# rsokolovskii/fl_scaling_sc_ldpc

Measured on AMD Instinct MI355X. Metric: MC codeword trials/sec, (4,8) SC-LDPC L=50 N=1000 eps=0.48 full BP, higher is better.
Workload: dtype u32

## Files before the change

fl_scaling_sc_ldpc_amd/csrc/philox.h:

```cpp
#pragma once
#include <cstdint>

namespace scldpc_dev {

__device__ __forceinline__ void philox4x32_10(uint32_t c0, uint32_t c1, uint32_t c2, uint32_t c3,
                                              uint32_t k0, uint32_t k1, uint32_t (&out)[4])
{
#pragma unroll
    for (int r = 0; r < 10; r++) {
        const uint64_t p0 = (uint64_t)0xD2511F53u * c0, p1 = (uint64_t)0xCD9E8D57u * c2;
        c0 = __builtin_amdgcn_bitop3_b32((uint32_t)(p1 >> 32), c1, k0, 0x96); c1 = (uint32_t)p1;
        c2 = __builtin_amdgcn_bitop3_b32((uint32_t)(p0 >> 32), c3, k1, 0x96); c3 = (uint32_t)p0;
        k0 += 0x9E3779B9u; k1 += 0xBB67AE85u;
    }
    out[0] = c0; out[1] = c1; out[2] = c2; out[3] = c3;
}

}
```

fl_scaling_sc_ldpc_amd/csrc/sampler_v2.hip:

```cpp
#include "common.h"
#include "kernel_util.h"
#include "philox.h"
#include <algorithm>
#include <cstdlib>

namespace {

using scldpc_dev::philox4x32_10;
using scldpc_dev::wave_inclusive_scan;

constexpr int kThreads = 1024;
constexpr int kWaves = kThreads / 64;
constexpr int kMaxDoped = 32;
constexpr int kWorkCap = 1024;

struct S2Args {
    int L, cns_pos, vns_pos, n, S, D, nb, nw;
    int ntrials;
    int force_exact;
    int ndoped;
    int doped[kMaxDoped];
    uint32_t seed_lo, seed_hi;
    unsigned long long trial0;
    uint32_t thresh;
    int off_gpk, off_fix, off_stage, off_wsum;
    uint16_t *vn_adj16;
    uint16_t *cn_adj16;
    uint32_t *chan;
};

template <int KMAX, int ROWS, int CNMODE, bool PERSIST = false>
__global__ __launch_bounds__(kThreads, KMAX == 1 ? 8 : 4) __attribute__((amdgpu_num_sgpr(72))) void sample_philox_v2_kernel(const S2Args a)
{
    constexpr int DV = 4, DC_SHIFT = 3, E = 4 * KMAX;
    constexpr int LG = ROWS == 1 ? 10 : ROWS == 2 ? 11 : ROWS == 4 ? 12 : 13;
    constexpr int KSHIFT = 32 - LG - 2;
    constexpr bool INCL = KMAX == 1;
    static_assert(ROWS * kThreads == (1 << LG) && (INCL ? ROWS <= 4 : ROWS == 8), "ROWS is 1, 2, 4 (KMAX 1) or 8 (KMAX 2)");
    extern __shared__ uint32_t lds[];
    uint32_t *hist = lds;
    uint32_t *gpk = lds + a.off_gpk;
    uint16_t *fix = reinterpret_cast<uint16_t *>(lds + a.off_fix);
    uint16_t *stage = reinterpret_cast<uint16_t *>(lds + a.off_stage);
    uint32_t *wsum = lds + a.off_wsum;
    uint32_t *wl = wsum + 32;

    const int tid = threadIdx.x, lane = tid & 63, wave = tid >> 6;
    const int S = a.S, nb = a.nb;
    const int ncalls = S >> 2;
    bool own[KMAX];
#pragma unroll
    for (int k = 0; k < KMAX; k++) own[k] = tid + k * kThreads < ncalls;
    auto sock = [&](int e) { return (uint32_t)((tid + (e >> 2) * kThreads) * 4 + (e & 3)); };
    auto stage_entry = [&](int p, uint32_t sck) -> uint16_t {
        const int u = (int)(sck & 3u), t = (int)(sck >> 2);
        if ((unsigned)(p - u) >= (unsigned)a.L) return (uint16_t)0xFFFFu;
        return CNMODE == 1 ? (uint16_t)((p - u) * a.vns_pos + t) : (uint16_t)sck;
    };

    auto nib_sum = [](uint32_t x) {
        const uint32_t v = (x & 0x0F0Fu) + ((x >> 4) & 0x0F0Fu);
        return (v + (v >> 8)) & 0xFFu;
    };
    auto load_words = [&](uint32_t (&x)[ROWS]) {
        if constexpr (ROWS % 4 == 0) {
#pragma unroll
            for (int r = 0; r < ROWS / 4; r++) {
                const uint4 q = reinterpret_cast<const uint4 *>(hist)[tid * (ROWS / 4) + r];
                x[4 * r] = q.x; x[4 * r + 1] = q.y; x[4 * r + 2] = q.z; x[4 * r + 3] = q.w;
            }
        } else if constexpr (ROWS == 2) { const uint2 q = reinterpret_cast<const uint2 *>(hist)[tid]; x[0] = q.x; x[1] = q.y; }
        else x[0] = hist[tid];
    };
    auto store_words = [&](const uint32_t (&x)[ROWS]) {
        if constexpr (ROWS % 4 == 0) {
#pragma unroll
            for (int r = 0; r < ROWS / 4; r++)
                reinterpret_cast<uint4 *>(hist)[tid * (ROWS / 4) + r] = make_uint4(x[4 * r], x[4 * r + 1], x[4 * r + 2], x[4 * r + 3]);
        } else if constexpr (ROWS == 2) reinterpret_cast<uint2 *>(hist)[tid] = make_uint2(x[0], x[1]);
        else hist[tid] = x[0];
    };
    STAMP_DECL
    for (int b = tid; b < nb; b += kThreads) hist[b] = 0;
    if (tid == 0) { wsum[kWaves] = 0; wsum[kWaves + 1] = 0; }
    __syncthreads();
    auto sample_trial = [&](const int tr) {
    const unsigned long long trial = a.trial0 + (unsigned long long)tr;
    const uint32_t t_lo = (uint32_t)trial, t_hi = (uint32_t)(trial >> 32);
    uint32_t rowP[KMAX], rowQ[KMAX], rowR[KMAX];
#pragma unroll
    for (int k = 0; k < KMAX; k++) rowP[k] = rowQ[k] = rowR[k] = 0;
    uint32_t nxt[E];
#pragma unroll
    for (int k = 0; k < KMAX; k++) {
        uint32_t r[4] = {0, 0, 0, 0};
        if (own[k]) philox4x32_10((uint32_t)(tid + k * kThreads), 0u, t_lo, t_hi, a.seed_lo, a.seed_hi, r);
#pragma unroll
        for (int u = 0; u < 4; u++) nxt[4 * k + u] = r[u];
    }
    for (int p = 0; p < a.D; p++) {
        STAMP(0);
        uint32_t key[E], slot[E], crowded = 0;
        auto word_of = [](uint32_t k) { return (k >> KSHIFT) & ~3u; };
        auto nib_of = [](uint32_t k) { return (k >> (KSHIFT - 2)) & 12u; };
#pragma unroll
        for (int e = 0; e < E; e++) {
            key[e] = nxt[e];
            const uint32_t sh = nib_of(key[e]);
            uint32_t *w = reinterpret_cast<uint32_t *>(reinterpret_cast<char *>(hist) + word_of(key[e]));
            slot[e] = (atomicAdd(w, (own[e >> 2] ? 1u : 0u) << sh) >> sh) & 0xFu;
            if constexpr (!INCL) crowded = max(crowded, slot[e]);
        }
        if (!INCL && crowded >= 15u) wsum[kWaves + 1] = 1u;
        __syncthreads();
        STAMP(1);

        bool ranked;
        if constexpr (INCL) {
            uint32_t x[ROWS], t20[ROWS], tot20 = 0;
            load_words(x);
#pragma unroll
            for (int r = 0; r < ROWS; r++) {
                x[r] *= 0x111110u;
                t20[r] = x[r] & 0xF00000u;
                tot20 += t20[r];
            }
            const uint32_t tot = tot20 >> 20, inc = wave_inclusive_scan(tot);
            if (lane == 63) wsum[wave] = inc;
            __syncthreads();
            uint32_t winc = lane < kWaves ? wsum[lane] : 0u;
            const uint32_t wt = winc;
            winc += (uint32_t)__builtin_amdgcn_update_dpp(0, (int)winc, 0x111, 0xF, 0xF, false);
            winc += (uint32_t)__builtin_amdgcn_update_dpp(0, (int)winc, 0x112, 0xF, 0xF, false);
            winc += (uint32_t)__builtin_amdgcn_update_dpp(0, (int)winc, 0x114, 0xF, 0xF, false);
            winc += (uint32_t)__builtin_amdgcn_update_dpp(0, (int)winc, 0x118, 0xF, 0xF, false);
            ranked = __builtin_amdgcn_readlane((int)winc, kWaves - 1) == S;
            uint32_t pre20 = (inc - tot + (uint32_t)__builtin_amdgcn_readlane((int)(winc - wt), wave)) << 20;
#pragma unroll
            for (int r = 0; r < ROWS; r++) {
                x[r] = (x[r] & 0xFFFF0u) | pre20;
                pre20 += t20[r];
            }
            store_words(x);
        } else {
            uint32_t x[ROWS], v[ROWS], tot = 0;
            load_words(x);
#pragma unroll
            for (int r = 0; r < ROWS; r++) v[r] = 0;
            if constexpr (ROWS % 2 == 0) {
#pragma unroll
                for (int r = 0; r < ROWS; r += 2) {
                    const uint32_t y = x[r] | (x[r + 1] << 16);
                    const uint32_t sb = (y & 0x0F0F0F0Fu) + ((y >> 4) & 0x0F0F0F0Fu);
                    v[r] = (sb & 0xFFu) + ((sb >> 8) & 0xFFu);
                    v[r + 1] = ((sb >> 16) & 0xFFu) + (sb >> 24);
                    tot += v[r] + v[r + 1];
                }
            } else {
                static_assert(ROWS == 1 || ROWS % 2 == 0, "ROWS is 1, 2, 4 or 8");
                v[0] = nib_sum(x[0]);
                tot = v[0];
            }
            const uint32_t inc = wave_inclusive_scan(tot);
            if (lane == 63) wsum[wave] = inc;
            __syncthreads();
            const uint32_t wt = lane < kWaves ? wsum[lane] : 0u;
            const uint32_t winc = wave_inclusive_scan(wt);
            uint32_t pre = inc - tot + (uint32_t)__builtin_amdgcn_readlane((int)(winc - wt), wave);
#pragma unroll
            for (int r = 0; r < ROWS; r++) { x[r] |= pre << 16; pre += v[r]; }
            store_words(x);
        }
        __syncthreads();
        if constexpr (!INCL) ranked = wsum[kWaves + 1] == 0u;
        STAMP(2);

        if (ranked) {
            uint32_t rk[E], g0a[E], g1a[E];
            bool st[E];
            if constexpr (INCL) {
                uint32_t h[E];
#pragma unroll
                for (int e = 0; e < E; e++) h[e] = *reinterpret_cast<const uint32_t *>(reinterpret_cast<const char *>(hist) + word_of(key[e]));
#pragma unroll
                for (int e = 0; e < E; e++) {
                    const uint32_t t = h[e] >> nib_of(key[e]), pre = h[e] >> 20;
                    g0a[e] = pre + (t & 0xFu);
                    g1a[e] = pre + ((t >> 4) & 0xFu);
                    rk[e] = g0a[e] + slot[e];
                    st[e] = own[e >> 2] && ((g0a[e] ^ (g1a[e] - 1u)) >> DC_SHIFT) != 0u;
                }
            } else {
                uint32_t h[E];
#pragma unroll
                for (int e = 0; e < E; e++) h[e] = hist[own[e >> 2] ? (key[e] >> KSHIFT) >> 2 : 0u];
#pragma unroll
                for (int e = 0; e < E; e++) {
                    const uint32_t k4 = ((key[e] >> KSHIFT) & 3u) * 4u, x = h[e];
                    const uint32_t below = x & ((1u << k4) - 1u);
                    g0a[e] = (x >> 16) + (below & 0xFu) + ((below >> 4) & 0xFu) + ((below >> 8) & 0xFu);
                    g1a[e] = g0a[e] + ((x >> k4) & 0xFu);
                    rk[e] = g0a[e] + slot[e];
                    st[e] = own[e >> 2] && ((g1a[e] - 1u) >> DC_SHIFT) != (g0a[e] >> DC_SHIFT);
                }
            }
            if constexpr (INCL) {
                unsigned long long vote[E], anyv = 0;
                int total = 0;
#pragma unroll
                for (int e = 0; e < E; e++) { vote[e] = __builtin_amdgcn_ballot_w64(st[e]); anyv |= vote[e]; total += __builtin_popcountll(vote[e]); }
                if (anyv) {
                    int base = 0;
                    if (lane == 0) base = atomicAdd(reinterpret_cast<int *>(&wsum[kWaves]), total);
                    base = __builtin_amdgcn_readfirstlane(base);
                    const bool fits = base + total <= kWorkCap;
#pragma unroll
                    for (int e = 0; e < E; e++) {
                        if (st[e]) {
                            const uint32_t w = __builtin_amdgcn_mbcnt_hi((uint32_t)(vote[e] >> 32),
                                                                         __builtin_amdgcn_mbcnt_lo((uint32_t)vote[e], (uint32_t)base));
                            const uint32_t pk = (key[e] << LG) | sock(e);
                            gpk[rk[e]] = pk;
                            if (fits) { wl[2 * w] = g0a[e] | (g1a[e] << 16); wl[2 * w + 1] = pk; }
                        }
                        base += __builtin_popcountll(vote[e]);
                    }
                }
            } else {
                uint32_t smask = 0;
#pragma unroll
                for (int e = 0; e < E; e++) smask |= (st[e] ? 1u : 0u) << e;
                while (smask) {
                    const uint32_t e = (uint32_t)__ffs((int)smask) - 1u;
                    smask &= smask - 1u;
                    uint32_t ky = key[0], r0 = rk[0], g0 = g0a[0], g1 = g1a[0];
#pragma unroll
                    for (int f = 1; f < E; f++)
                        if (e == (uint32_t)f) { ky = key[f]; r0 = rk[f]; g0 = g0a[f]; g1 = g1a[f]; }
                    const uint32_t pk = (ky << LG) | (uint32_t)((tid + (int)(e >> 2) * kThreads) * 4 + (int)(e & 3u));
                    gpk[r0] = pk;
                    const int w = atomicAdd(reinterpret_cast<int *>(&wsum[kWaves]), 1);
                    if (w < kWorkCap) { wl[2 * w] = g0 | (g1 << 16); wl[2 * w + 1] = pk; }
                }
            }
#pragma unroll
            for (int k = 0; k < KMAX; k++) {
                if (!own[k]) continue;
                uint2 v;
                v.x = (rk[4 * k] >> DC_SHIFT) | ((rk[4 * k + 1] >> DC_SHIFT) << 16);
                v.y = (rk[4 * k + 2] >> DC_SHIFT) | ((rk[4 * k + 3] >> DC_SHIFT) << 16);
                reinterpret_cast<uint2 *>(fix)[tid + k * kThreads] = v;
            }
            if constexpr (CNMODE != 0) {
#pragma unroll
                for (int k = 0; k < KMAX; k++) {
                    if (!own[k]) continue;
#pragma unroll
                    for (int u = 0; u < 4; u++) stage[rk[4 * k + u]] = stage_entry(p, sock(4 * k + u));
                }
            }
        }
        __syncthreads();
        STAMP(3);

        {
            uint32_t z[ROWS];
#pragma unroll
            for (int r = 0; r < ROWS; r++) z[r] = 0;
            store_words(z);
            int nwork = (int)wsum[kWaves];
            const bool exact = !ranked || nwork > kWorkCap || a.force_exact == p || a.force_exact == -2;
            if (exact) {
                asm volatile("; ledger: cold");
                nwork = 0;
#pragma unroll
                for (int e = 0; e < E; e++) if (own[e >> 2]) gpk[sock(e)] = key[e];
                __syncthreads();
                uint32_t xr[E];
#pragma unroll
                for (int e = 0; e < E; e++) xr[e] = 0;
                for (int s2 = 0; s2 < S; s2++) {
                    const uint32_t k2 = gpk[s2];
#pragma unroll
                    for (int e = 0; e < E; e++) xr[e] += (k2 < key[e]) || (k2 == key[e] && (uint32_t)s2 < sock(e));
                }
#pragma unroll
                for (int k = 0; k < KMAX; k++) {
                    if (!own[k]) continue;
                    uint2 v;
                    v.x = (xr[4 * k] >> DC_SHIFT) | ((xr[4 * k + 1] >> DC_SHIFT) << 16);
                    v.y = (xr[4 * k + 2] >> DC_SHIFT) | ((xr[4 * k + 3] >> DC_SHIFT) << 16);
                    reinterpret_cast<uint2 *>(fix)[tid + k * kThreads] = v;
                    if constexpr (CNMODE != 0) {
#pragma unroll
                        for (int u = 0; u < 4; u++) stage[xr[4 * k + u]] = stage_entry(p, sock(4 * k + u));
                    }
                }
            }
            for (int w = tid; w < nwork; w += kThreads) {
                const uint32_t ea = wl[2 * w], pk = wl[2 * w + 1];
                uint32_t r = ea & 0xFFFFu;
#pragma unroll 1
                for (uint32_t m = ea & 0xFFFFu; m < (ea >> 16); m++) r += gpk[m] < pk;
                const uint32_t sck = pk & ((1u << LG) - 1u);
                if constexpr (CNMODE != 0) stage[r] = stage_entry(p, sck);
                fix[sck] = (uint16_t)(r >> DC_SHIFT);
            }
        }
        if (p + 1 < a.D) {
            uint32_t k_lo = a.seed_lo, k_hi = a.seed_hi;
            asm volatile("" : "+s"(k_lo), "+s"(k_hi));
#pragma unroll
            for (int k = 0; k < KMAX; k++) {
                uint32_t r[4] = {0, 0, 0, 0};
                if (own[k]) philox4x32_10((uint32_t)(tid + k * kThreads), (uint32_t)(p + 1), t_lo, t_hi, k_lo, k_hi, r);
#pragma unroll
                for (int u = 0; u < 4; u++) nxt[4 * k + u] = r[u];
            }
        }
        __syncthreads();
        if (tid == 0) { wsum[kWaves] = 0; wsum[kWaves + 1] = 0; }
        STAMP(4);

        const int qpos = p - (DV - 1);
#pragma unroll
        for (int k = 0; k < KMAX; k++) {
            uint2 c = make_uint2(0u, 0u);
            if (own[k]) c = reinterpret_cast<const uint2 *>(fix)[tid + k * kThreads];
            if (qpos >= 0 && own[k]) {
                const size_t j = (size_t)tr * a.n + (size_t)qpos * a.vns_pos + (size_t)(tid + k * kThreads);
                uint2 v;
                v.x = rowP[k];
                v.y = (rowR[k] >> 16) | (c.y & 0xFFFF0000u);
                reinterpret_cast<uint2 *>(a.vn_adj16)[j] = v;
            }
            rowP[k] = rowQ[k];
            rowQ[k] = (rowR[k] & 0xFFFFu) | (c.x & 0xFFFF0000u);
            rowR[k] = (c.x & 0xFFFFu) | (c.y << 16);
        }
        if constexpr (CNMODE != 0) {
            uint2 *dst = reinterpret_cast<uint2 *>(a.cn_adj16) + ((size_t)tr * a.D + p) * (size_t)(S >> 2);
            const uint2 *src = reinterpret_cast<const uint2 *>(stage);
            for (int w = tid; w < (S >> 2); w += kThreads) dst[w] = src[w];
        }
        STAMP(5);
    }

    uint32_t *chan = a.chan + (size_t)tr * a.nw;
    for (int w = tid; w < a.nw; w += kThreads) {
        uint32_t word = 0;
#pragma unroll
        for (int c = 0; c < 8; c++) {
            uint32_t r[4];
            philox4x32_10((uint32_t)(w * 8 + c), 0x80000000u, t_lo, t_hi, a.seed_lo, a.seed_hi, r);
#pragma unroll
            for (int u = 0; u < 4; u++) word |= (uint32_t)((r[u] >> 1) < a.thresh) << (c * 4 + u);
        }
        const int j0 = w * 32;
        if (j0 + 32 > a.n) word &= (1u << (a.n - j0)) - 1u;
        for (int d = 0; d < a.ndoped; d++) {
            const int lo = max(a.doped[d] * a.vns_pos, j0) - j0, hi = min((a.doped[d] + 1) * a.vns_pos, j0 + 32) - j0;
            if (lo < hi) word &= ~(((hi - lo) == 32 ? 0xFFFFFFFFu : ((1u << (hi - lo)) - 1u)) << lo);
        }
        chan[w] = word;
    }
    STAMP(6);
    };
    if constexpr (PERSIST) {
        for (int tr = blockIdx.x; tr < a.ntrials; tr += gridDim.x) {
            sample_trial(tr);
            __syncthreads();
        }
    } else {
        sample_trial((int)blockIdx.x);
    }
    STAMP_FLUSH();
}


__device__ __forceinline__ uint32_t wl_entry_vn(const S2Args &a, int p, uint32_t sck)
{
    return (uint32_t)((p - (int)(sck & 3u)) * a.vns_pos + (int)(sck >> 2));
}

template <int LG, int CNMODE>
__global__ __launch_bounds__(kThreads, 8) __attribute__((amdgpu_num_sgpr(72))) void sample_philox_v3_kernel(const S2Args a)
{
    constexpr int DV = 4, DC_SHIFT = 3, E = 4;
    constexpr int NB = 1 << LG, ROWS = NB / kThreads;
    constexpr int KSHIFT = 32 - LG - 2;
    constexpr uint32_t LOWMASK = (1u << KSHIFT) - 1u;
    constexpr int SBITS = LG;
    static_assert(ROWS == 1 || ROWS == 2 || ROWS == 4, "one Philox call per thread: at most 4096 sockets per position");
    extern __shared__ uint32_t lds[];
    uint32_t *hist0 = lds;
    uint32_t *gpk = lds + a.off_gpk;
    uint16_t *fix = reinterpret_cast<uint16_t *>(lds + a.off_fix);
    uint16_t *stage = reinterpret_cast<uint16_t *>(lds + a.off_stage);
    uint32_t *wsum = lds + a.off_wsum;
    uint32_t *wl = wsum + 32;

    const int tid = threadIdx.x, lane = tid & 63, wave = tid >> 6;
    const int S = a.S;
    const bool own = tid < (S >> 2);
    const unsigned long long trial = a.trial0 + blockIdx.x;
    const uint32_t t_lo = (uint32_t)trial, t_hi = (uint32_t)(trial >> 32);
    const int tr = blockIdx.x;

    STAMP_DECL
    for (int b = tid; b < 2 * NB; b += kThreads) hist0[b] = 0;
    if (tid < 32) wsum[tid] = 0;
    __syncthreads();

    uint32_t rowP = 0, rowQ = 0, rowR = 0;
    uint32_t key[E] = {0, 0, 0, 0}, slot[E] = {0, 0, 0, 0};
    uint32_t ent0 = CNMODE == 1 ? (uint32_t)tid : (uint32_t)(4 * tid);
    uint32_t vV = (uint32_t)a.vns_pos;
    asm volatile("" : "+v"(vV));

    for (int p = 0; p <= a.D; p++) {
        uint32_t *hc = hist0 + (p & 1) * NB, *hp = hist0 + ((p & 1) ^ 1) * NB;
        const bool live = p < a.D;
        STAMP(0);
        if (p > 0) {
            int nwork = (int)wsum[16];
            const bool exact = wsum[18 + ((p - 1) & 1)] != 0u || nwork > kWorkCap || a.force_exact == p - 1 || a.force_exact == -2;
            if (exact) {
                uint32_t k2[4] = {0, 0, 0, 0};
                uint32_t f_lo = a.seed_lo, f_hi = a.seed_hi;
                asm volatile("" : "+s"(f_lo), "+s"(f_hi));
                if (own) philox4x32_10((uint32_t)tid, (uint32_t)(p - 1), t_lo, t_hi, f_lo, f_hi, k2);
                if (own) { gpk[4 * tid] = k2[0]; gpk[4 * tid + 1] = k2[1]; gpk[4 * tid + 2] = k2[2]; gpk[4 * tid + 3] = k2[3]; }
                __syncthreads();
                uint32_t xr[4] = {0, 0, 0, 0};
                for (int s2 = 0; s2 < S; s2++) {
                    const uint32_t kk = gpk[s2];
#pragma unroll
                    for (int u = 0; u < 4; u++) xr[u] += (kk < k2[u]) || (kk == k2[u] && s2 < 4 * tid + u);
                }
                if (own) {
                    uint2 v;
                    v.x = (xr[0] >> DC_SHIFT) | ((xr[1] >> DC_SHIFT) << 16);
                    v.y = (xr[2] >> DC_SHIFT) | ((xr[3] >> DC_SHIFT) << 16);
                    reinterpret_cast<uint2 *>(fix)[tid] = v;
                    if constexpr (CNMODE != 0) {
#pragma unroll
                        for (int u = 0; u < 4; u++) {
                            const int pu = p - 1 - u;
                            stage[xr[u]] = (unsigned)pu < (unsigned)a.L ? (uint16_t)(CNMODE == 1 ? pu * a.vns_pos + tid : 4 * tid + u) : (uint16_t)0xFFFFu;
                        }
                    }
                }
                nwork = 0;
            }
            for (int w = tid; w < nwork; w += kThreads) {
                const uint32_t ea = wl[2 * w], pk = wl[2 * w + 1];
                const uint32_t g0 = ea & 0xFFFFu, cnt = (ea >> 16) & 0xFu, sl = (ea >> 20) & 0xFu;
                uint32_t r = g0;
                for (uint32_t m = 0; m < cnt; m++)
                    if (m != sl) r += gpk[g0 + m] < pk;
                const uint32_t sck = pk & ((1u << SBITS) - 1u);
                if constexpr (CNMODE != 0) stage[r] = (uint16_t)(ea >> 24 ? 0xFFFFu : (CNMODE == 1 ? wl_entry_vn(a, p - 1, sck) : sck));
                fix[sck] = (uint16_t)(r >> DC_SHIFT);
            }
            {
                if constexpr (ROWS == 4) reinterpret_cast<uint4 *>(hp)[tid] = make_uint4(0u, 0u, 0u, 0u);
                else if constexpr (ROWS == 2) reinterpret_cast<uint2 *>(hp)[tid] = make_uint2(0u, 0u);
                else hp[tid] = 0u;
            }
        }
        STAMP(1);
        if (live) {
            {
                uint32_t k_lo = a.seed_lo, k_hi = a.seed_hi;
                asm volatile("" : "+s"(k_lo), "+s"(k_hi));
                uint32_t r[4] = {0, 0, 0, 0};
                if (own) philox4x32_10((uint32_t)tid, (uint32_t)p, t_lo, t_hi, k_lo, k_hi, r);
#pragma unroll
                for (int u = 0; u < 4; u++) key[u] = r[u];
            }
            uint32_t crowded = 0;
#pragma unroll
            for (int e = 0; e < E; e++) {
                const uint32_t boff = (key[e] >> KSHIFT) & ~3u, sh = (key[e] >> (KSHIFT - 2)) & 12u;
                const uint32_t old = atomicAdd(reinterpret_cast<uint32_t *>(reinterpret_cast<char *>(hc) + boff), (own ? 16u : 0u) << sh);
                slot[e] = (old >> (sh + 4u)) & 0xFu;
                crowded |= slot[e] + 1u;
            }
            if (crowded & 16u) wsum[18 + (p & 1)] = 1u;
        }
        STAMP(2);
        __syncthreads();
        STAMP(3);
        if (tid == 0) { wsum[16] = 0; wsum[18 + ((p & 1) ^ 1)] = 0; }
        if (live) {
            uint32_t x[ROWS], tot = 0, over = 0;
            if constexpr (ROWS == 4) { const uint4 q = reinterpret_cast<const uint4 *>(hc)[tid]; x[0] = q.x; x[1] = q.y; x[2] = q.z; x[3] = q.w; }
            else if constexpr (ROWS == 2) { const uint2 q = reinterpret_cast<const uint2 *>(hc)[tid]; x[0] = q.x; x[1] = q.y; }
            else x[0] = hc[tid];
            uint32_t v[ROWS];
#pragma unroll
            for (int r = 0; r < ROWS; r++) {
                const uint32_t y = x[r] * 0x1111u;
                const uint32_t sb = (x[r] & 0x0F0F0u) + ((x[r] >> 4) & 0x0F0F0u);
                v[r] = ((sb + (sb >> 8)) >> 4) & 0xFFu;
                over |= v[r];
                x[r] = y & 0xFFFF0u;
                tot += v[r];
            }
            if (over & ~15u) wsum[18 + (p & 1)] = 1u;
            const uint32_t inc = wave_inclusive_scan(tot);
            uint32_t pre = inc - tot;
#pragma unroll
            for (int r = 0; r < ROWS; r++) { x[r] |= pre << 20; pre += v[r]; }
            if constexpr (ROWS == 4) reinterpret_cast<uint4 *>(hc)[tid] = make_uint4(x[0], x[1], x[2], x[3]);
            else if constexpr (ROWS == 2) reinterpret_cast<uint2 *>(hc)[tid] = make_uint2(x[0], x[1]);
            else hc[tid] = x[0];
            if (lane == 63) wsum[wave] = inc;
        }
        if (p > 0) {
            const int pp = p - 1, qpos = pp - (DV - 1);
            uint2 c = make_uint2(0u, 0u);
            if (own) c = reinterpret_cast<const uint2 *>(fix)[tid];
            if (qpos >= 0 && own) {
                const size_t j = (size_t)tr * a.n + (size_t)qpos * a.vns_pos + (size_t)tid;
                uint2 vv;
                vv.x = rowP;
                vv.y = (rowR >> 16) | (c.y & 0xFFFF0000u);
                reinterpret_cast<uint2 *>(a.vn_adj16)[j] = vv;
            }
            rowP = rowQ;
            rowQ = (rowR & 0xFFFFu) | (c.x & 0xFFFF0000u);
            rowR = (c.x & 0xFFFFu) | (c.y << 16);
            if constexpr (CNMODE != 0) {
                uint2 *dst = reinterpret_cast<uint2 *>(a.cn_adj16) + ((size_t)tr * a.D + pp) * (size_t)(S >> 2);
                const uint2 *src = reinterpret_cast<const uint2 *>(stage);
                if (own) dst[tid] = src[tid];
            }
        }
        STAMP(4);
        __syncthreads();
        STAMP(5);
        if (live && wsum[18 + (p & 1)] == 0u) {
            const uint32_t wt = lane < kWaves ? wsum[lane] : 0u;
            uint32_t wi = wt;
            wi += (uint32_t)__builtin_amdgcn_update_dpp(0, (int)wi, 0x111, 0xF, 0xF, false);
            wi += (uint32_t)__builtin_amdgcn_update_dpp(0, (int)wi, 0x112, 0xF, 0xF, false);
            wi += (uint32_t)__builtin_amdgcn_update_dpp(0, (int)wi, 0x114, 0xF, 0xF, false);
            wi += (uint32_t)__builtin_amdgcn_update_dpp(0, (int)wi, 0x118, 0xF, 0xF, false);
            const uint32_t wex = wi - wt;
            uint32_t h[E], wb[E], rk[E], g0a[E], cnta[E];
#pragma unroll
            for (int e = 0; e < E; e++) h[e] = *reinterpret_cast<const uint32_t *>(reinterpret_cast<const char *>(hc) + ((key[e] >> KSHIFT) & ~3u));
#pragma unroll
            for (int e = 0; e < E; e++) wb[e] = (uint32_t)__builtin_amdgcn_ds_bpermute((int)((key[e] >> 26) & 0x3Cu), (int)wex);
            bool st[E];
            bool anyst = false;
#pragma unroll
            for (int e = 0; e < E; e++) {
                const uint32_t t1 = h[e] >> ((key[e] >> (KSHIFT - 2)) & 12u);
                const uint32_t excl = t1 & 15u, incl = (t1 >> 4) & 15u;
                g0a[e] = (h[e] >> 20) + wb[e] + excl;
                cnta[e] = incl - excl;
                rk[e] = g0a[e] + slot[e];
                st[e] = own && ((g0a[e] ^ (g0a[e] + cnta[e] - 1u)) >> DC_SHIFT) != 0u;
                anyst = anyst || st[e];
            }
            if (own) {
                uint2 vv;
                vv.x = (rk[0] >> DC_SHIFT) | ((rk[1] >> DC_SHIFT) << 16);
                vv.y = (rk[2] >> DC_SHIFT) | ((rk[3] >> DC_SHIFT) << 16);
                reinterpret_cast<uint2 *>(fix)[tid] = vv;
            }
            const bool edge = p < DV - 1 || p >= a.L;
            if constexpr (CNMODE != 0) {
                if (own) {
                    uint32_t ent[E];
                    ent[0] = ent0;
#pragma unroll
                    for (int u = 1; u < 4; u++) ent[u] = CNMODE == 1 ? ent[u - 1] - vV : ent[u - 1] + 1u;
                    if (!edge) {
#pragma unroll
                        for (int u = 0; u < 4; u++) stage[rk[u]] = (uint16_t)ent[u];
                    } else {
#pragma unroll
                        for (int u = 0; u < 4; u++) stage[rk[u]] = (unsigned)(p - u) < (unsigned)a.L ? (uint16_t)ent[u] : (uint16_t)0xFFFFu;
                    }
                }
            }
            if (__builtin_amdgcn_ballot_w64(anyst)) {
                unsigned long long vote[E];
                int total = 0;
#pragma unroll
                for (int e = 0; e < E; e++) { vote[e] = __builtin_amdgcn_ballot_w64(st[e]); total += __builtin_popcountll(vote[e]); }
                int base = 0;
                if (lane == 0) base = atomicAdd(reinterpret_cast<int *>(&wsum[16]), total);
                base = __builtin_amdgcn_readfirstlane(base);
#pragma unroll
                for (int e = 0; e < E; e++) {
                    if (st[e]) {
                        const int w = base + (int)__builtin_amdgcn_mbcnt_hi((uint32_t)(vote[e] >> 32), __builtin_amdgcn_mbcnt_lo((uint32_t)vote[e], 0u));
                        const uint32_t pk = ((key[e] & LOWMASK) << SBITS) | (uint32_t)(4 * tid + e);
                        gpk[g0a[e] + slot[e]] = pk;
                        const uint32_t none = CNMODE != 0 && edge && !((unsigned)(p - e) < (unsigned)a.L) ? 1u : 0u;
                        if (w < kWorkCap) { wl[2 * w] = g0a[e] | (cnta[e] << 16) | (slot[e] << 20) | (none << 24); wl[2 * w + 1] = pk; }
                    }
                    base += __builtin_popcountll(vote[e]);
                }
            }
        }
        if constexpr (CNMODE == 1) ent0 += vV;
        STAMP(6);
        __syncthreads();
        STAMP(7);
    }

    uint32_t *chan = a.chan + (size_t)tr * a.nw;
    for (int w = tid; w < a.nw; w += kThreads) {
        uint32_t word = 0;
        uint32_t c_lo = a.seed_lo, c_hi = a.seed_hi;
        asm volatile("" : "+s"(c_lo), "+s"(c_hi));
#pragma unroll
        for (int c = 0; c < 8; c++) {
            uint32_t r[4];
            philox4x32_10((uint32_t)(w * 8 + c), 0x80000000u, t_lo, t_hi, c_lo, c_hi, r);
#pragma unroll
            for (int u = 0; u < 4; u++) word |= (uint32_t)((r[u] >> 1) < a.thresh) << (c * 4 + u);
        }
        const int j0 = w * 32;
        if (j0 + 32 > a.n) word &= (1u << (a.n - j0)) - 1u;
        for (int d = 0; d < a.ndoped; d++) {
            const int lo = max(a.doped[d] * a.vns_pos, j0) - j0, hi = min((a.doped[d] + 1) * a.vns_pos, j0 + 32) - j0;
            if (lo < hi) word &= ~(((hi - lo) == 32 ? 0xFFFFFFFFu : ((1u << (hi - lo)) - 1u)) << lo);
        }
        chan[w] = word;
    }
    STAMP(8);
    STAMP_FLUSH();
}

int launch_v2(const char *who, int cnmode, const scldpc_code_params *p, uint64_t seed, uint64_t trial0, int32_t ntrials,
              double eps, int32_t ndoped, const int32_t *doped_positions, uint16_t *d_vn_adj16, uint16_t *d_table,
              uint32_t *d_chan_bits, void *stream)
{
    if (ntrials < 0 || (ntrials > 0 && (!d_vn_adj16 || !d_chan_bits)))
        return scldpc::set_error(SCLDPC_ERR_BAD_ARG, "%s: null buffer or negative ntrials", who);
    if (ndoped < 0 || ndoped > kMaxDoped || (ndoped > 0 && !doped_positions))
        return scldpc::set_error(SCLDPC_ERR_BAD_ARG, "%s: 0 <= ndoped <= %d", who, kMaxDoped);
    if (!(eps >= 0.0 && eps <= 1.0))
        return scldpc::set_error(SCLDPC_ERR_BAD_ARG, "%s: eps=%g outside [0,1]", who, eps);
    if (ntrials == 0) return SCLDPC_OK;
    if (!d_table) cnmode = 0;

    S2Args a{};
    a.L = p->L; a.cns_pos = p->cns_pos; a.vns_pos = p->vns_pos;
    a.n = scldpc::n_of(p); a.S = p->cns_pos * p->dc; a.D = p->L + p->dv - 1; a.nw = scldpc::nw_of(p);
    int lg = 10;
    while ((1 << lg) < a.S) lg++;
    a.nb = 1 << lg;
    a.ndoped = ndoped;
    for (int d = 0; d < ndoped; d++) {
        if (doped_positions[d] < 0 || doped_positions[d] >= p->L)
            return scldpc::set_error(SCLDPC_ERR_BAD_ARG, "doped position %d outside [0,%d)", doped_positions[d], p->L);
        a.doped[d] = doped_positions[d];
    }
    a.seed_lo = (uint32_t)seed; a.seed_hi = (uint32_t)(seed >> 32);
    a.trial0 = trial0;
    {
        const double x = eps * 2147483647.0;
        double c = (double)(uint64_t)x;
        if (c < x) c += 1.0;
        a.thresh = (uint32_t)c;
    }
    const char *gen_env = getenv("SCLDPC_SAMPLER_GEN");
    const bool v3 = a.nb <= 4 * kThreads && gen_env && atoi(gen_env) == 3;
    int off = ((v3 ? 2 : 1) * a.nb + 3) & ~3;
    a.off_gpk = off;   off += (a.S + 3) & ~3;
    a.off_fix = off;   off += (a.S / 2 + 3) & ~3;
    a.off_stage = off; off += cnmode ? (a.S / 2 + 3) & ~3 : 0;
    a.off_wsum = off;  off += 32 + 2 * kWorkCap;
    size_t lds_bytes = 4u * (size_t)off;
    lds_bytes = std::min(lds_bytes + scldpc::debug_lds_pad("SAMPLER"), std::max(lds_bytes, (size_t)scldpc::kMaxLdsBytes));
    if (lds_bytes > (size_t)scldpc::kMaxLdsBytes)
        return scldpc::set_error(SCLDPC_ERR_TOO_LARGE, "%s: %zu bytes of LDS per trial", who, lds_bytes);
    a.vn_adj16 = d_vn_adj16; a.cn_adj16 = d_table; a.chan = d_chan_bits;
    a.ntrials = ntrials;
    a.force_exact = -1;
    if (const char *v = getenv("SCLDPC_DEBUG_SAMPLER_EXACT_POS")) a.force_exact = atoi(v);

    using Kern = void (*)(const S2Args);
    static const Kern table[4][3] = {
        {sample_philox_v2_kernel<1, 1, 0>, sample_philox_v2_kernel<1, 1, 1>, sample_philox_v2_kernel<1, 1, 2>},
        {sample_philox_v2_kernel<1, 2, 0>, sample_philox_v2_kernel<1, 2, 1>, sample_philox_v2_kernel<1, 2, 2>},
        {sample_philox_v2_kernel<1, 4, 0>, sample_philox_v2_kernel<1, 4, 1>, sample_philox_v2_kernel<1, 4, 2>},
        {sample_philox_v2_kernel<2, 8, 0>, sample_philox_v2_kernel<2, 8, 1>, sample_philox_v2_kernel<2, 8, 2>},
    };
    const int rows = a.nb / kThreads;
    static const Kern table3[3][3] = {
        {sample_philox_v3_kernel<10, 0>, sample_philox_v3_kernel<10, 1>, sample_philox_v3_kernel<10, 2>},
        {sample_philox_v3_kernel<11, 0>, sample_philox_v3_kernel<11, 1>, sample_philox_v3_kernel<11, 2>},
        {sample_philox_v3_kernel<12, 0>, sample_philox_v3_kernel<12, 1>, sample_philox_v3_kernel<12, 2>},
    };
    const int grid = v3 ? ntrials : scldpc::debug_grid("SAMPLER", ntrials);
    Kern kern = v3 ? table3[lg - 10][cnmode] : table[rows == 1 ? 0 : rows == 2 ? 1 : rows == 4 ? 2 : 3][cnmode];
    if (grid < ntrials && rows == 4 && cnmode == 1) kern = sample_philox_v2_kernel<1, 4, 1, true>;
    else if (grid < ntrials) return scldpc::set_error(SCLDPC_ERR_BAD_ARG, "SCLDPC_DEBUG_GRID_SAMPLER: only the <1,4,1> kernel has a persistent form");
    if (int rc_ = scldpc::allow_max_lds(reinterpret_cast<const void *>(kern))) return rc_;
    hipLaunchKernelGGL(kern, dim3(grid), dim3(kThreads), lds_bytes, static_cast<hipStream_t>(stream), a);
    SCLDPC_HIP_CHECK(hipGetLastError());
    return SCLDPC_OK;
}

bool v2_shape(const scldpc_code_params *p)
{
    if (scldpc::check_params(p)) return false;
    const int S = p->cns_pos * p->dc;
    return p->dv == 4 && p->dc == 8 && (S & 3) == 0 && S <= 8192 && p->vns_pos * p->dv == S;
}

}

extern "C" int scldpc_sample_philox_cn16_supported(const scldpc_code_params *p)
{
    return v2_shape(p) && scldpc::n_of(p) < 65535;
}

extern "C" int scldpc_sample_philox_sock16_supported(const scldpc_code_params *p)
{
    return v2_shape(p);
}

extern "C" int scldpc_sample_philox_device_cn16(const scldpc_code_params *p, uint64_t seed, uint64_t trial0,
                                                int32_t ntrials, double eps, int32_t ndoped,
                                                const int32_t *doped_positions, uint16_t *d_vn_adj16,
                                                uint16_t *d_cn_adj16, uint32_t *d_chan_bits, void *stream)
{
    const char *who = "scldpc_sample_philox_device_cn16";
    if (int rc = scldpc::check_params(p)) return rc;
    if (!scldpc_sample_philox_cn16_supported(p))
        return scldpc::set_error(SCLDPC_ERR_TOO_LARGE, "%s: takes dv = 4, dc = 8, at most 8192 sockets per position and "
                                 "fewer than 65535 VNs (got dv=%d dc=%d cns_pos=%d n=%d)", who, p->dv, p->dc, p->cns_pos,
                                 scldpc::n_of(p));
    return launch_v2(who, 1, p, seed, trial0, ntrials, eps, ndoped, doped_positions, d_vn_adj16, d_cn_adj16, d_chan_bits,
                     stream);
}

extern "C" int scldpc_sample_philox_device_sock16(const scldpc_code_params *p, uint64_t seed, uint64_t trial0,
                                                  int32_t ntrials, double eps, int32_t ndoped,
                                                  const int32_t *doped_positions, uint16_t *d_vn_adj16,
                                                  uint16_t *d_cn_sock16, uint32_t *d_chan_bits, void *stream)
{
    const char *who = "scldpc_sample_philox_device_sock16";
    if (int rc = scldpc::check_params(p)) return rc;
    if (!scldpc_sample_philox_sock16_supported(p))
        return scldpc::set_error(SCLDPC_ERR_TOO_LARGE, "%s: takes dv = 4, dc = 8 and at most 8192 sockets per position "
                                 "(got dv=%d dc=%d cns_pos=%d)", who, p->dv, p->dc, p->cns_pos);
    return launch_v2(who, 2, p, seed, trial0, ntrials, eps, ndoped, doped_positions, d_vn_adj16, d_cn_sock16, d_chan_bits,
                     stream);
}
```

Baseline: 1.214 million.

## Hoist per-thread Philox prefix rounds and share trial-uniform rounds across positions

Splits Philox4x32-10 into a per-thread prefix (depends only on thread counter, trial and key), a wave-uniform part that depends on the position counter, and a tail for rounds 3-9. The prefix is computed once per trial and reused across all D positions, so each position pays for fewer per-thread rounds while producing the same random stream. It also makes the LDS layout offsets compile-time for the inclusive path, and uses a hand-written ds_add_rtn with a ballot-masked worklist append. It adds a raw asm LDS atomic with an explicit waitcnt and changes the host layout sizing, which must stay consistent with the constexpr offsets.

```diff
diff --git a/fl_scaling_sc_ldpc_amd/csrc/philox.h b/fl_scaling_sc_ldpc_amd/csrc/philox.h
--- a/fl_scaling_sc_ldpc_amd/csrc/philox.h
+++ b/fl_scaling_sc_ldpc_amd/csrc/philox.h
@@ -1,17 +1,86 @@
 #pragma once
 #include <cstdint>
 
+#if defined(__HIPCC__) || defined(__CUDACC__)
+#define SCLDPC_PHILOX_HD __host__ __device__ __forceinline__
+#else
+#define SCLDPC_PHILOX_HD inline
+#endif
+
 namespace scldpc_dev {
 
-__device__ __forceinline__ void philox4x32_10(uint32_t c0, uint32_t c1, uint32_t c2, uint32_t c3,
-                                              uint32_t k0, uint32_t k1, uint32_t (&out)[4])
+constexpr uint32_t kPhiloxM0 = 0xD2511F53u, kPhiloxM1 = 0xCD9E8D57u;
+constexpr uint32_t kPhiloxW0 = 0x9E3779B9u, kPhiloxW1 = 0xBB67AE85u;
+
+SCLDPC_PHILOX_HD uint32_t philox_xor3(uint32_t a, uint32_t b, uint32_t c)
+{
+#if defined(__HIP_DEVICE_COMPILE__)
+    return __builtin_amdgcn_bitop3_b32(a, b, c, 0x96);
+#else
+    return a ^ b ^ c;
+#endif
+}
+
+SCLDPC_PHILOX_HD void philox4x32_10(uint32_t c0, uint32_t c1, uint32_t c2, uint32_t c3,
+                                    uint32_t k0, uint32_t k1, uint32_t (&out)[4])
 {
 #pragma unroll
     for (int r = 0; r < 10; r++) {
-        const uint64_t p0 = (uint64_t)0xD2511F53u * c0, p1 = (uint64_t)0xCD9E8D57u * c2;
-        c0 = __builtin_amdgcn_bitop3_b32((uint32_t)(p1 >> 32), c1, k0, 0x96); c1 = (uint32_t)p1;
-        c2 = __builtin_amdgcn_bitop3_b32((uint32_t)(p0 >> 32), c3, k1, 0x96); c3 = (uint32_t)p0;
-        k0 += 0x9E3779B9u; k1 += 0xBB67AE85u;
+        const uint64_t p0 = (uint64_t)kPhiloxM0 * c0, p1 = (uint64_t)kPhiloxM1 * c2;
+        c0 = philox_xor3((uint32_t)(p1 >> 32), c1, k0); c1 = (uint32_t)p1;
+        c2 = philox_xor3((uint32_t)(p0 >> 32), c3, k1); c3 = (uint32_t)p0;
+        k0 += kPhiloxW0; k1 += kPhiloxW1;
+    }
+    out[0] = c0; out[1] = c1; out[2] = c2; out[3] = c3;
+}
+
+struct PhiloxPrefix {
+    uint32_t c3r1;
+    uint32_t a;
+    uint32_t b, c;
+};
+struct PhiloxUniform {
+    uint32_t u;
+    uint32_t v;
+};
+
+SCLDPC_PHILOX_HD PhiloxPrefix philox_prefix(uint32_t c0, uint32_t c2, uint32_t c3, uint32_t k0, uint32_t k1)
+{
+    const uint64_t p0 = (uint64_t)kPhiloxM0 * c0;
+    const uint32_t c1r1 = (uint32_t)((uint64_t)kPhiloxM1 * c2);
+    const uint32_t c2r1 = philox_xor3((uint32_t)(p0 >> 32), c3, k1);
+    const uint64_t p1 = (uint64_t)kPhiloxM1 * c2r1;
+    const uint32_t c0r2 = philox_xor3((uint32_t)(p1 >> 32), c1r1, k0 + kPhiloxW0);
+    const uint64_t q0 = (uint64_t)kPhiloxM0 * c0r2;
+    PhiloxPrefix f;
+    f.c3r1 = (uint32_t)p0;
+    f.a = (uint32_t)p1 ^ (k0 + 2u * kPhiloxW0);
+    f.b = (uint32_t)(q0 >> 32);
+    f.c = (uint32_t)q0;
+    return f;
+}
+
+SCLDPC_PHILOX_HD PhiloxUniform philox_uniform(uint32_t c1, uint32_t c2, uint32_t k0, uint32_t k1)
+{
+    const uint32_t c0r1 = (uint32_t)(((uint64_t)kPhiloxM1 * c2) >> 32) ^ c1 ^ k0;
+    const uint64_t p0 = (uint64_t)kPhiloxM0 * c0r1;
+    PhiloxUniform g;
+    g.u = (uint32_t)(p0 >> 32) ^ (k1 + kPhiloxW1);
+    g.v = (uint32_t)p0 ^ (k1 + 2u * kPhiloxW1);
+    return g;
+}
+
+SCLDPC_PHILOX_HD void philox_tail(const PhiloxPrefix &f, const PhiloxUniform &g, uint32_t k0, uint32_t k1, uint32_t (&out)[4])
+{
+    const uint64_t q1 = (uint64_t)kPhiloxM1 * (g.u ^ f.c3r1);
+    uint32_t c0 = (uint32_t)(q1 >> 32) ^ f.a, c1 = (uint32_t)q1, c2 = f.b ^ g.v, c3 = f.c;
+    k0 += 3u * kPhiloxW0; k1 += 3u * kPhiloxW1;
+#pragma unroll
+    for (int r = 3; r < 10; r++) {
+        const uint64_t p0 = (uint64_t)kPhiloxM0 * c0, p1 = (uint64_t)kPhiloxM1 * c2;
+        c0 = philox_xor3((uint32_t)(p1 >> 32), c1, k0); c1 = (uint32_t)p1;
+        c2 = philox_xor3((uint32_t)(p0 >> 32), c3, k1); c3 = (uint32_t)p0;
+        k0 += kPhiloxW0; k1 += kPhiloxW1;
     }
     out[0] = c0; out[1] = c1; out[2] = c2; out[3] = c3;
 }
diff --git a/fl_scaling_sc_ldpc_amd/csrc/sampler_v2.hip b/fl_scaling_sc_ldpc_amd/csrc/sampler_v2.hip
--- a/fl_scaling_sc_ldpc_amd/csrc/sampler_v2.hip
+++ b/fl_scaling_sc_ldpc_amd/csrc/sampler_v2.hip
@@ -7,12 +7,25 @@
 namespace {
 
 using scldpc_dev::philox4x32_10;
+using scldpc_dev::philox_prefix;
+using scldpc_dev::philox_tail;
+using scldpc_dev::philox_uniform;
+using scldpc_dev::PhiloxPrefix;
+using scldpc_dev::PhiloxUniform;
 using scldpc_dev::wave_inclusive_scan;
 
 constexpr int kThreads = 1024;
 constexpr int kWaves = kThreads / 64;
 constexpr int kMaxDoped = 32;
 constexpr int kWorkCap = 1024;
+
+__device__ __forceinline__ uint32_t lds_add_rtn(uint32_t *p, uint32_t v)
+{
+    const uint32_t addr = (uint32_t)(uintptr_t)(__attribute__((address_space(3))) uint32_t *)p;
+    uint32_t old;
+    asm volatile("ds_add_rtn_u32 %0, %1, %2\n\ts_waitcnt lgkmcnt(0)" : "=v"(old) : "v"(addr), "v"(v) : "memory");
+    return old;
+}
 
 struct S2Args {
     int L, cns_pos, vns_pos, n, S, D, nb, nw;
@@ -29,6 +42,13 @@
     uint32_t *chan;
 };
 
+template <int ROWS, int CNMODE>
+struct V2Layout {
+    static constexpr int nb = ROWS * kThreads;
+    static constexpr int off_gpk = nb, off_fix = off_gpk + nb, off_stage = off_fix + nb / 2;
+    static constexpr int off_wsum = off_stage + (CNMODE != 0 ? nb / 2 : 0);
+};
+
 template <int KMAX, int ROWS, int CNMODE, bool PERSIST = false>
 __global__ __launch_bounds__(kThreads, KMAX == 1 ? 8 : 4) __attribute__((amdgpu_num_sgpr(72))) void sample_philox_v2_kernel(const S2Args a)
 {
@@ -38,15 +58,18 @@
     constexpr bool INCL = KMAX == 1;
     static_assert(ROWS * kThreads == (1 << LG) && (INCL ? ROWS <= 4 : ROWS == 8), "ROWS is 1, 2, 4 (KMAX 1) or 8 (KMAX 2)");
     extern __shared__ uint32_t lds[];
+    using Lay = V2Layout<ROWS, CNMODE>;
+    const int off_gpk = INCL ? Lay::off_gpk : a.off_gpk, off_fix = INCL ? Lay::off_fix : a.off_fix;
+    const int off_stage = INCL ? Lay::off_stage : a.off_stage, off_wsum = INCL ? Lay::off_wsum : a.off_wsum;
     uint32_t *hist = lds;
-    uint32_t *gpk = lds + a.off_gpk;
-    uint16_t *fix = reinterpret_cast<uint16_t *>(lds + a.off_fix);
-    uint16_t *stage = reinterpret_cast<uint16_t *>(lds + a.off_stage);
-    uint32_t *wsum = lds + a.off_wsum;
+    uint32_t *gpk = lds + off_gpk;
+    uint16_t *fix = reinterpret_cast<uint16_t *>(lds + off_fix);
+    uint16_t *stage = reinterpret_cast<uint16_t *>(lds + off_stage);
+    uint32_t *wsum = lds + off_wsum;
     uint32_t *wl = wsum + 32;
 
-    const int tid = threadIdx.x, lane = tid & 63, wave = tid >> 6;
-    const int S = a.S, nb = a.nb;
+    const int tid = threadIdx.x, lane = tid & 63, wave = __builtin_amdgcn_readfirstlane(tid >> 6);
+    const int S = a.S, nb = INCL ? ROWS * kThreads : a.nb;
     const int ncalls = S >> 2;
     bool own[KMAX];
 #pragma unroll
@@ -90,13 +113,19 @@
     uint32_t rowP[KMAX], rowQ[KMAX], rowR[KMAX];
 #pragma unroll
     for (int k = 0; k < KMAX; k++) rowP[k] = rowQ[k] = rowR[k] = 0;
+    PhiloxPrefix pre[KMAX];
+#pragma unroll
+    for (int k = 0; k < KMAX; k++) pre[k] = philox_prefix((uint32_t)(tid + k * kThreads), t_lo, t_hi, a.seed_lo, a.seed_hi);
     uint32_t nxt[E];
-#pragma unroll
-    for (int k = 0; k < KMAX; k++) {
-        uint32_t r[4] = {0, 0, 0, 0};
-        if (own[k]) philox4x32_10((uint32_t)(tid + k * kThreads), 0u, t_lo, t_hi, a.seed_lo, a.seed_hi, r);
-#pragma unroll
-        for (int u = 0; u < 4; u++) nxt[4 * k + u] = r[u];
+    {
+        const PhiloxUniform un = philox_uniform(0u, t_lo, a.seed_lo, a.seed_hi);
+#pragma unroll
+        for (int k = 0; k < KMAX; k++) {
+            uint32_t r[4] = {0, 0, 0, 0};
+            if (own[k]) philox_tail(pre[k], un, a.seed_lo, a.seed_hi, r);
+#pragma unroll
+            for (int u = 0; u < 4; u++) nxt[4 * k + u] = r[u];
+        }
     }
     for (int p = 0; p < a.D; p++) {
         STAMP(0);
@@ -177,7 +206,7 @@
 
         if (ranked) {
             uint32_t rk[E], g0a[E], g1a[E];
-            bool st[E];
+            bool st[E], sx[E];
             if constexpr (INCL) {
                 uint32_t h[E];
 #pragma unroll
@@ -188,7 +217,8 @@
                     g0a[e] = pre + (t & 0xFu);
                     g1a[e] = pre + ((t >> 4) & 0xFu);
                     rk[e] = g0a[e] + slot[e];
-                    st[e] = own[e >> 2] && ((g0a[e] ^ (g1a[e] - 1u)) >> DC_SHIFT) != 0u;
+                    sx[e] = ((g0a[e] ^ (g1a[e] - 1u)) >> DC_SHIFT) != 0u;
+                    st[e] = own[e >> 2] && sx[e];
                 }
             } else {
                 uint32_t h[E];
@@ -205,25 +235,33 @@
                 }
             }
             if constexpr (INCL) {
-                unsigned long long vote[E], anyv = 0;
+                const unsigned long long ownv = __builtin_amdgcn_ballot_w64(own[0]);
+                unsigned long long vote[E];
                 int total = 0;
 #pragma unroll
-                for (int e = 0; e < E; e++) { vote[e] = __builtin_amdgcn_ballot_w64(st[e]); anyv |= vote[e]; total += __builtin_popcountll(vote[e]); }
-                if (anyv) {
-                    int base = 0;
-                    if (lane == 0) base = atomicAdd(reinterpret_cast<int *>(&wsum[kWaves]), total);
-                    base = __builtin_amdgcn_readfirstlane(base);
-                    const bool fits = base + total <= kWorkCap;
-#pragma unroll
-                    for (int e = 0; e < E; e++) {
-                        if (st[e]) {
-                            const uint32_t w = __builtin_amdgcn_mbcnt_hi((uint32_t)(vote[e] >> 32),
-                                                                         __builtin_amdgcn_mbcnt_lo((uint32_t)vote[e], (uint32_t)base));
-                            const uint32_t pk = (key[e] << LG) | sock(e);
-                            gpk[rk[e]] = pk;
-                            if (fits) { wl[2 * w] = g0a[e] | (g1a[e] << 16); wl[2 * w + 1] = pk; }
+                for (int e = 0; e < E; e++) { vote[e] = __builtin_amdgcn_ballot_w64(sx[e]) & ownv; total += __builtin_popcountll(vote[e]); }
+                if (total != 0) {
+                    uint32_t ln, got = 0;
+                    asm volatile("v_and_b32 %0, 63, %1" : "=v"(ln) : "v"(tid));
+                    if (ln == 0u) got = lds_add_rtn(&wsum[kWaves], (uint32_t)total);
+                    int base = __builtin_amdgcn_readfirstlane((int)got);
+                    if (base + total <= kWorkCap) {
+                        static_assert((Lay::off_wsum + 32) % 2 == 0, "the worklist starts on a word pair");
+                        uint2 *wl2 = reinterpret_cast<uint2 *>(lds);
+                        base += (Lay::off_wsum + 32) / 2;
+#pragma unroll
+                        for (int e = 0; e < E; e++) {
+                            if (st[e]) {
+                                const uint32_t w = __builtin_amdgcn_mbcnt_hi((uint32_t)(vote[e] >> 32),
+                                                                             __builtin_amdgcn_mbcnt_lo((uint32_t)vote[e], (uint32_t)base));
+                                const uint32_t pk = (key[e] << LG) | sock(e);
+                                gpk[rk[e]] = pk;
+                                uint32_t *ent = reinterpret_cast<uint32_t *>(wl2 + w);
+                                ent[0] = g0a[e] | (g1a[e] << 16);
+                                ent[1] = pk;
+                            }
+                            base += __builtin_popcountll(vote[e]);
                         }
-                        base += __builtin_popcountll(vote[e]);
                     }
                 }
             } else {
@@ -309,11 +347,13 @@
         }
         if (p + 1 < a.D) {
             uint32_t k_lo = a.seed_lo, k_hi = a.seed_hi;
-            asm volatile("" : "+s"(k_lo), "+s"(k_hi));
+            uint32_t tl = t_lo;
+            asm volatile("" : "+s"(k_lo), "+s"(k_hi), "+s"(tl));
+            const PhiloxUniform un = philox_uniform((uint32_t)(p + 1), tl, k_lo, k_hi);
 #pragma unroll
             for (int k = 0; k < KMAX; k++) {
                 uint32_t r[4] = {0, 0, 0, 0};
-                if (own[k]) philox4x32_10((uint32_t)(tid + k * kThreads), (uint32_t)(p + 1), t_lo, t_hi, k_lo, k_hi, r);
+                if (own[k]) philox_tail(pre[k], un, k_lo, k_hi, r);
 #pragma unroll
                 for (int u = 0; u < 4; u++) nxt[4 * k + u] = r[u];
             }
@@ -328,7 +368,7 @@
             uint2 c = make_uint2(0u, 0u);
             if (own[k]) c = reinterpret_cast<const uint2 *>(fix)[tid + k * kThreads];
             if (qpos >= 0 && own[k]) {
-                const size_t j = (size_t)tr * a.n + (size_t)qpos * a.vns_pos + (size_t)(tid + k * kThreads);
+                const size_t j = (size_t)tr * a.n + (size_t)((uint32_t)qpos * (uint32_t)a.vns_pos + (uint32_t)(tid + k * kThreads));
                 uint2 v;
                 v.x = rowP[k];
                 v.y = (rowR[k] >> 16) | (c.y & 0xFFFF0000u);
@@ -347,12 +387,13 @@
     }
 
     uint32_t *chan = a.chan + (size_t)tr * a.nw;
+    const PhiloxUniform chun = philox_uniform(0x80000000u, t_lo, a.seed_lo, a.seed_hi);
     for (int w = tid; w < a.nw; w += kThreads) {
         uint32_t word = 0;
 #pragma unroll
         for (int c = 0; c < 8; c++) {
             uint32_t r[4];
-            philox4x32_10((uint32_t)(w * 8 + c), 0x80000000u, t_lo, t_hi, a.seed_lo, a.seed_hi, r);
+            philox_tail(philox_prefix((uint32_t)(w * 8 + c), t_lo, t_hi, a.seed_lo, a.seed_hi), chun, a.seed_lo, a.seed_hi, r);
 #pragma unroll
             for (int u = 0; u < 4; u++) word |= (uint32_t)((r[u] >> 1) < a.thresh) << (c * 4 + u);
         }
@@ -674,10 +715,11 @@
     }
     const char *gen_env = getenv("SCLDPC_SAMPLER_GEN");
     const bool v3 = a.nb <= 4 * kThreads && gen_env && atoi(gen_env) == 3;
+    const int s_lay = !v3 && a.nb <= 4 * kThreads ? a.nb : a.S;
     int off = ((v3 ? 2 : 1) * a.nb + 3) & ~3;
-    a.off_gpk = off;   off += (a.S + 3) & ~3;
-    a.off_fix = off;   off += (a.S / 2 + 3) & ~3;
-    a.off_stage = off; off += cnmode ? (a.S / 2 + 3) & ~3 : 0;
+    a.off_gpk = off;   off += (s_lay + 3) & ~3;
+    a.off_fix = off;   off += (s_lay / 2 + 3) & ~3;
+    a.off_stage = off; off += cnmode ? (s_lay / 2 + 3) & ~3 : 0;
     a.off_wsum = off;  off += 32 + 2 * kWorkCap;
     size_t lds_bytes = 4u * (size_t)off;
     lds_bytes = std::min(lds_bytes + scldpc::debug_lds_pad("SAMPLER"), std::max(lds_bytes, (size_t)scldpc::kMaxLdsBytes));
```

Result: faster. 1.246 million (median of 6 runs) (+2.6%).
